# ModelCloud/GPTQModel

Hardware: NVIDIA H100
Metric: W4A16 g128 QuantLinear: decode tok/s + prefill TFLOPS vs HBM/TC roofline (higher is better)
Workload: dtype f16

## Files before the change

### gptqmodel_b200/csrc/b2q_api.cu

```cuda
#include <cstdarg>
#include <cstdio>
#include <cstdlib>

#include "../../include/b2q.h"
#include "b2q_internal.h"

namespace b2q {
static thread_local char g_err[512] = "";

void set_error(const char* fmt, ...) {
  va_list ap;
  va_start(ap, fmt);
  vsnprintf(g_err, sizeof(g_err), fmt, ap);
  va_end(ap);
}

static int env_int(const char* name, int dflt) {
  const char* e = getenv(name);
  return (e != nullptr && e[0] != 0) ? atoi(e) : dflt;
}

static EnvCfg read_env() {
  EnvCfg c;
  c.disable_pdl = env_int("B2Q_DISABLE_PDL", 0);
  c.midm = env_int("B2Q_MIDM", 1);
  c.decode_blocks_m = env_int("B2Q_DECODE_BLOCKS_M", 0);
  c.decode_groups2 = env_int("B2Q_DECODE_GROUPS", 1) == 2;
  c.decode_v2 = env_int("B2Q_DECODE_V2", -1);
  c.decode2_gw = env_int("B2Q_DECODE2_GW", 0);
  c.decode2_ks = env_int("B2Q_DECODE2_KS", 0);
  c.decode2_xtma = env_int("B2Q_DECODE2_XTMA", 0);
  c.decode2_fastsync = env_int("B2Q_DECODE2_FASTSYNC", 0);
  c.midm_ks = env_int("B2Q_MIDM_KS", 0);
  c.midm_dqg1 = env_int("B2Q_MIDM_DQG1", 0);
  return c;
}

int num_sms() {
  static int cache[32] = {};
  int dev = 0;
  if (cudaGetDevice(&dev) != cudaSuccess || dev < 0 || dev >= 32) {
    (void)cudaGetLastError();
    return 132;
  }
  if (cache[dev] == 0) {
    int n = 0;
    if (cudaDeviceGetAttribute(&n, cudaDevAttrMultiProcessorCount, dev) != cudaSuccess || n <= 0) {
      (void)cudaGetLastError();
      n = 132;
    }
    cache[dev] = n < 160 ? n : 160;
  }
  return cache[dev];
}

static EnvCfg g_env = read_env();
const EnvCfg& env() { return g_env; }
void reload_env() { g_env = read_env(); }

struct DeviceGuard {
  int prev = -1, dev = -1;
  explicit DeviceGuard(const void* p) {
    cudaPointerAttributes at;
    if (p != nullptr && cudaPointerGetAttributes(&at, p) == cudaSuccess && at.type == cudaMemoryTypeDevice) {
      dev = at.device;
      if (cudaGetDevice(&prev) == cudaSuccess && prev != dev) cudaSetDevice(dev);
      else prev = -1;
    }
    (void)cudaGetLastError();
  }
  ~DeviceGuard() {
    if (prev >= 0) cudaSetDevice(prev);
  }
};

static int check_cuda(int e, const char* what) {
  if (e > 0) set_error("%s: CUDA error %d (%s)", what, e, cudaGetErrorString((cudaError_t)e));
  return e;
}

static int validate(const char* fn, const void* x, const void* packed, const void* scales, const void* out, int M,
                    int K, int N, int bits, int group_size, int dtype) {
  if (x == nullptr || packed == nullptr || scales == nullptr || out == nullptr) {
    set_error("%s: null pointer argument", fn);
    return -2;
  }
  if (bits != 4 && bits != 8) {
// ... 467 lines not shown
```

### gptqmodel_b200/csrc/b2q_gemm.cu

```cuda
#include <cuda.h>

#include "b2q_common.cuh"
#include "b2q_dequant.cuh"
#include "b2q_gemm.cuh"
#include "b2q_internal.h"
#include "b2q_wgmma.cuh"

namespace b2q {

template <typename T, int BITS, bool ASYM, int STAGES>
__global__ void __launch_bounds__(G_THREADS, 1)
    gemm_kernel(const __grid_constant__ CUtensorMap tmap_x, const __grid_constant__ GemmSets S, int M, int K,
                int gshc) {
  using C = GemmCfg<BITS, STAGES>;
  using E = ET<T>;
  extern __shared__ uint8_t smem_raw[];
  const uint32_t smem_base = (smem_u32(smem_raw) + 1023u) & ~1023u;
  uint8_t* smem = smem_raw + (smem_base - smem_u32(smem_raw));

  const uint32_t sA = smem_base;
  const uint32_t sB = sA + STAGES * C::A_BYTES;
  const uint32_t sP = sB + STAGES * C::B_BYTES;
  const uint32_t sBar = sP + STAGES * C::P_BYTES;
  const uint32_t bar_full = sBar, bar_bready = sBar + 8 * STAGES, bar_empty = sBar + 16 * STAGES;

  int set = 0, tn = blockIdx.x;
  if (S.nsets > 1 && tn >= S.tn_end[0]) {
    set = (S.nsets > 2 && tn >= S.tn_end[1]) ? 2 : 1;
    tn -= S.tn_end[set - 1];
  }
  const int N = S.N[set];
  const uint4* __restrict__ packed = S.packed[set];
  const T* __restrict__ scales = reinterpret_cast<const T*>(S.scales[set]);
  const uint32_t* __restrict__ qzeros = S.qzeros[set];

  const int warp = threadIdx.x >> 5, lane = threadIdx.x & 31;
  const int NT = N >> 5;
  const int n0 = tn * G_BN, m0 = blockIdx.y * G_BM;
  const int nt0 = n0 >> 5;
  const int ntiles = min(4, NT - nt0);
  const int nkb = K / G_BK;

  if (threadIdx.x == 0) {
    prefetch_tmap(&tmap_x);
    for (int s = 0; s < STAGES; ++s) {
      mbar_init(bar_full + 8 * s, 1);
      mbar_init(bar_bready + 8 * s, G_DQ_THREADS);
      mbar_init(bar_empty + 8 * s, 1);
    }
    fence_mbar_init();
  }
  __syncthreads();

  if (warp == 8) {
    if (lane == 0) {
      const int FT = N >> 4, ft0 = n0 >> 4;
      const uint32_t pbytes4 = (uint32_t)min(8, FT - ft0) * 512u;
      const uint32_t pbytes8 = (uint32_t)ntiles * C::SUB * 512u;
      for (int kb = 0; kb < nkb; ++kb) {
        const int s = kb % STAGES;
        const uint32_t ph = (kb / STAGES) & 1;
        mbar_wait(bar_empty + 8 * s, ph ^ 1);
        const int g0 = (2 * kb) >> gshc, g1 = (2 * kb + 1) >> gshc;
        const int nrows = (g1 != g0) ? 2 : 1;
        const uint32_t sbytes = (uint32_t)min(G_BN, N - n0) * 2u, zbytes = ASYM ? sbytes / 4u : 0u;
        mbar_expect_tx(bar_full + 8 * s,
                       C::A_BYTES + (BITS == 4 ? pbytes4 + nrows * (sbytes + zbytes) : 2 * pbytes8));
        tma_load_2d(sA + s * C::A_BYTES, &tmap_x, bar_full + 8 * s, kb * G_BK, m0);
        if (BITS == 4) {
          bulk_load(sP + s * C::P_BYTES, packed + ((size_t)kb * FT + ft0) * 32, pbytes4, bar_full + 8 * s);
          for (int r = 0; r < nrows; ++r) {
            const int gr = r ? g1 : g0;
            bulk_load(sP + s * C::P_BYTES + 4096 + r * 320, scales + (size_t)gr * N + n0, sbytes, bar_full + 8 * s);
            if (ASYM)
              bulk_load(sP + s * C::P_BYTES + 4096 + r * 320 + 256, qzeros + (size_t)gr * (N >> 3) + (n0 >> 3),
                        zbytes, bar_full + 8 * s);
          }
        } else {
#pragma unroll
          for (int j = 0; j < 2; ++j)
            bulk_load(sP + s * C::P_BYTES + j * C::P_CHUNK_BYTES,
                      packed + ((size_t)(kb * 2 + j) * NT + nt0) * C::SUB * 32, pbytes8, bar_full + 8 * s);
        }
      }
    }
  } else if (warp < 4) {
    float acc[2][G_BN / 2];
#pragma unroll
    for (int mb = 0; mb < 2; ++mb)
#pragma unroll
      for (int i = 0; i < G_BN / 2; ++i) acc[mb][i] = 0.f;
    for (int kb = 0; kb < nkb; ++kb) {
      const int s = kb % STAGES;
      const uint32_t ph = (kb / STAGES) & 1;
      mbar_wait(bar_full + 8 * s, ph);
      mbar_wait(bar_bready + 8 * s, ph);
      wgmma_fence();
      const uint64_t bdesc = wgmma_desc_k_sw128(sB + s * C::B_BYTES);
      const uint64_t adesc = wgmma_desc_k_sw128(sA + s * C::A_BYTES);
#pragma unroll
      for (int k = 0; k < G_BK / 16; ++k) {
#pragma unroll
        for (int mb = 0; mb < 2; ++mb)
          Wgmma<E::FMT, G_BN>::mma(acc[mb], adesc + 512 * mb + 2 * k, bdesc + 2 * k, (kb | k) != 0 ? 1u : 0u);
      }
      wgmma_commit();
      wgmma_wait<1>();
      if (kb > 0 && threadIdx.x == 0) mbar_arrive(bar_empty + 8 * ((kb - 1) % STAGES));
    }
    wgmma_wait<0>();
#pragma unroll
    for (int mb = 0; mb < 2; ++mb) wgmma_fence_regs(acc[mb]);

    const T* __restrict__ bias = reinterpret_cast<const T*>(S.bias[set]);
    T* __restrict__ out = reinterpret_cast<T*>(S.out[set]);
#pragma unroll
    for (int mb = 0; mb < 2; ++mb) {
#pragma unroll
      for (int h = 0; h < 2; ++h) {
        const int row = m0 + 64 * mb + 16 * warp + (lane >> 2) + 8 * h;
        if (row >= M) continue;
        T* dst = out + (size_t)row * N;
#pragma unroll
        for (int j = 0; j < G_BN / 8; ++j) {
          const int col = n0 + 8 * j + 2 * (lane & 3);
          if (col >= N) continue;
          float f0 = acc[mb][4 * j + 2 * h], f1 = acc[mb][4 * j + 2 * h + 1];
          if (bias != nullptr) {
            f0 = E::to_f(E::from_f(f0)) + E::to_f(bias[col]);
            f1 = E::to_f(E::from_f(f1)) + E::to_f(bias[col + 1]);
          }
          *reinterpret_cast<uint32_t*>(dst + col) = E::pack2(f0, f1);
        }
      }
    }
  } else {
    const int t = threadIdx.x - G_MMA_THREADS;
    constexpr int PF = 32 / BITS;
    constexpr int ZSYM = 1 << (BITS - 1);
    if (BITS == 4) {
      const int lp = t & 31, g = lp >> 2, tt = lp & 3;
      int f[4];
      f[0] = (t >> 5) * 16 + g;
      f[1] = f[0] + 8;
      f[2] = f[0] + 64;
      f[3] = f[0] + 72;
      for (int kb = 0; kb < nkb; ++kb) {
        const int s = kb % STAGES;
        const uint32_t ph = (kb / STAGES) & 1;
        mbar_wait(bar_full + 8 * s, ph);
        const uint8_t* pst = smem + (sP - smem_base) + s * C::P_BYTES;
        const uint4* pj = reinterpret_cast<const uint4*>(pst);
        const int grow = ((2 * kb + (tt >> 1)) >> gshc) - ((2 * kb) >> gshc);
        const uint8_t* srow = pst + 4096 + grow * 320;
#pragma unroll
        for (int u = 0; u < 2; ++u) {
          const uint4 pv = pj[t + u * 128];
          const uint32_t s_lo = *reinterpret_cast<const uint16_t*>(srow + f[2 * u] * 2);
          const uint32_t s_hi = *reinterpret_cast<const uint16_t*>(srow + f[2 * u + 1] * 2);
          int zl = ZSYM, zh = ZSYM;
          if (ASYM) {
            const uint32_t zwl = *reinterpret_cast<const uint32_t*>(srow + 256 + (f[2 * u] >> 3) * 4);
            const uint32_t zwh = *reinterpret_cast<const uint32_t*>(srow + 256 + (f[2 * u + 1] >> 3) * 4);
            zl = (int)((zwl >> (4 * g)) & 15u);
            zh = (int)((zwh >> (4 * g)) & 15u);
          }
          uint4 lo[2], hi[2];
          Dequant<T, 4>::run(pv, s_lo, zl, s_hi, zh, lo, hi);
          const uint32_t sw = (uint32_t)g;
          const uint32_t rlo = sB + s * C::B_BYTES + f[2 * u] * 128;
          const uint32_t rhi = rlo + 8 * 128;
#pragma unroll
          for (int c = 0; c < 2; ++c) {
            const uint32_t off = (((uint32_t)(2 * tt + c)) ^ sw) << 4;
            asm volatile("st.shared.v4.u32 [%0], {%1,%2,%3,%4};" ::"r"(rlo + off), "r"(lo[c].x), "r"(lo[c].y),
                         "r"(lo[c].z), "r"(lo[c].w)
                         : "memory");
            asm volatile("st.shared.v4.u32 [%0], {%1,%2,%3,%4};" ::"r"(rhi + off), "r"(hi[c].x), "r"(hi[c].y),
                         "r"(hi[c].z), "r"(hi[c].w)
                         : "memory");
          }
        }
        fence_proxy_async_smem();
        mbar_arrive(bar_bready + 8 * s);
      }
    } else {
      const int n = n0 + t;
      const int nsafe = (n < N) ? n : 0;
      const int ntl = t >> 5;
      SZRaw cur[2], nxt[2];
      cur[0] = load_sz<T, BITS, ASYM>(scales, qzeros, 0, nsafe, N);
      cur[1] = load_sz<T, BITS, ASYM>(scales, qzeros, 1 >> gshc, nsafe, N);
      for (int kb = 0; kb < nkb; ++kb) {
        const int s = kb % STAGES;
        const uint32_t ph = (kb / STAGES) & 1;
        if (kb + 1 < nkb) {
          nxt[0] = load_sz<T, BITS, ASYM>(scales, qzeros, (2 * kb + 2) >> gshc, nsafe, N);
          nxt[1] = load_sz<T, BITS, ASYM>(scales, qzeros, (2 * kb + 3) >> gshc, nsafe, N);
        }
        mbar_wait(bar_full + 8 * s, ph);
        const uint32_t brow = sB + s * C::B_BYTES + t * 128;
        const uint32_t sw = (uint32_t)(t & 7);
#pragma unroll
        for (int j = 0; j < 2; ++j) {
          int z = ZSYM;
          if (ASYM) z = (int)((cur[j].zw >> (BITS * (nsafe % PF))) & ((1u << BITS) - 1));
          const uint4* pj = reinterpret_cast<const uint4*>(smem + (sP - smem_base) + s * C::P_BYTES +
                                                           j * C::P_CHUNK_BYTES);
#pragma unroll
          for (int h = 0; h < 2; ++h) {
            const uint4 pv = pj[(ntl * 2 + h) * 32 + lane];
            uint4 o[2];
            Dequant<T, 8>::run(pv, cur[j].s, z, o);
#pragma unroll
            for (int c = 0; c < 2; ++c) {
              const uint32_t addr = brow + (((uint32_t)(j * 4 + h * 2 + c) ^ sw) << 4);
              asm volatile("st.shared.v4.u32 [%0], {%1,%2,%3,%4};" ::"r"(addr), "r"(o[c].x), "r"(o[c].y),
                           "r"(o[c].z), "r"(o[c].w)
                           : "memory");
            }
          }
        }
        fence_proxy_async_smem();
        mbar_arrive(bar_bready + 8 * s);
        cur[0] = nxt[0];
        cur[1] = nxt[1];
      }
    }
  }
}

typedef CUresult (*EncodeTiledFn)(CUtensorMap*, CUtensorMapDataType, cuuint32_t, void*, const cuuint64_t*,
                                  const cuuint64_t*, const cuuint32_t*, const cuuint32_t*, CUtensorMapInterleave,
                                  CUtensorMapSwizzle, CUtensorMapL2promotion, CUtensorMapFloatOOBfill);

static EncodeTiledFn get_encode_fn() {
  static EncodeTiledFn fn = nullptr;
  if (fn == nullptr) {
    void* p = nullptr;
    cudaDriverEntryPointQueryResult qres;
    if (cudaGetDriverEntryPoint("cuTensorMapEncodeTiled", &p, cudaEnableDefault, &qres) == cudaSuccess &&
        qres == cudaDriverEntryPointSuccess)
      fn = reinterpret_cast<EncodeTiledFn>(p);
  }
  return fn;
}

int make_x_tmap_box(CUtensorMap* map, const void* x, int M, int K, int dtype, int box_rows) {
  struct Entry {
    const void* x;
    int M, K, dtype, box;
    CUtensorMap map;
  };
  constexpr int NCACHE = 16;
  static thread_local Entry cache[NCACHE];
  static thread_local int next = 0, filled = 0;
  for (int i = 0; i < filled; ++i) {
    const Entry& c = cache[i];
    if (c.x == x && c.M == M && c.K == K && c.dtype == dtype && c.box == box_rows) {
      *map = c.map;
      return 0;
    }
  }
  EncodeTiledFn enc = get_encode_fn();
  if (enc == nullptr) {
    set_error("b2q_gemm: cuTensorMapEncodeTiled not available from the driver");
    return -1;
  }
  cuuint64_t gdim[2] = {(cuuint64_t)K, (cuuint64_t)M};
  cuuint64_t gstride[1] = {(cuuint64_t)K * 2};
  cuuint32_t box[2] = {(cuuint32_t)G_BK, (cuuint32_t)box_rows};
  cuuint32_t estr[2] = {1, 1};
  CUresult r = enc(map, dtype == 0 ? CU_TENSOR_MAP_DATA_TYPE_FLOAT16 : CU_TENSOR_MAP_DATA_TYPE_BFLOAT16, 2,
                   const_cast<void*>(x), gdim, gstride, box, estr, CU_TENSOR_MAP_INTERLEAVE_NONE,
                   CU_TENSOR_MAP_SWIZZLE_128B, CU_TENSOR_MAP_L2_PROMOTION_L2_256B,
                   CU_TENSOR_MAP_FLOAT_OOB_FILL_NONE);
  if (r != CUDA_SUCCESS) {
    set_error("b2q_gemm: cuTensorMapEncodeTiled failed (%d) for x=%p M=%d K=%d box=%d", (int)r, x, M, K, box_rows);
    return -1;
  }
  Entry& e = cache[next];
  e.x = x;
  e.M = M;
  e.K = K;
  e.dtype = dtype;
  e.box = box_rows;
  e.map = *map;
  next = (next + 1) % NCACHE;
  if (filled < NCACHE) ++filled;
  return 0;
}

int make_x_tmap(CUtensorMap* map, const void* x, int M, int K, int dtype) {
  return make_x_tmap_box(map, x, M, K, dtype, 128);
}

int gemm_gshc(const MmArgs& a) {
  if (a.group_size == 32) return 0;
  if (a.group_size == 64) return 1;
  if (a.group_size == 128) return 2;
  return 31;
}


template <typename T, int BITS, bool ASYM, int STAGES>
static int launch_gemm_t(const MmArgs& a, const void* x, const GemmSets& S) {
  using C = GemmCfg<BITS, STAGES>;
  CUtensorMap tmap;
  if (make_x_tmap(&tmap, x, a.M, a.K, a.dtype) != 0) return -1;
  auto kern = gemm_kernel<T, BITS, ASYM, STAGES>;
  static uint32_t smem_ok = 0;
  if (int e = ensure_dyn_smem(kern, C::SMEM_BYTES, smem_ok, "b2q_gemm")) return e;
  dim3 grid(S.tn_end[S.nsets - 1], (a.M + G_BM - 1) / G_BM, 1);
  kern<<<grid, G_THREADS, C::SMEM_BYTES, a.stream>>>(tmap, S, a.M, a.K, gemm_gshc(a));
  return (int)cudaGetLastError();
}

static int launch_gemm_sets(const MmArgs& a, const void* x, const GemmSets& S) {
  const bool asym = S.qzeros[0] != nullptr;
#define B2Q_GEMM_CASE(T, BITS, ST) \
  (asym ? launch_gemm_t<T, BITS, true, ST>(a, x, S) : launch_gemm_t<T, BITS, false, ST>(a, x, S))
  if (a.dtype == 0) return a.bits == 4 ? B2Q_GEMM_CASE(__half, 4, 4) : B2Q_GEMM_CASE(__half, 8, 4);
  return a.bits == 4 ? B2Q_GEMM_CASE(__nv_bfloat16, 4, 4) : B2Q_GEMM_CASE(__nv_bfloat16, 8, 4);
#undef B2Q_GEMM_CASE
}

int launch_gemm_multi(const MmArgs& a, const void* x, int nsets, const void* const* packed, const void* const* scales,
                      const int32_t* const* qzeros, const void* const* bias, void* const* out, const int* Ns) {
  if (nsets < 1 || nsets > G_MAX_SETS) {
    set_error("b2q_gemm_multi: nsets=%d out of range (1..%d)", nsets, G_MAX_SETS);
    return -1;
  }
  if (a.K % G_BK != 0) {
    set_error("b2q_gemm_multi: K=%d must be a multiple of %d", a.K, G_BK);
    return -1;
  }
  GemmSets S = {};
  S.nsets = nsets;
  int tn = 0;
  for (int i = 0; i < nsets; ++i) {
    if (Ns[i] <= 0 || Ns[i] % 32 != 0 || packed[i] == nullptr || scales[i] == nullptr || out[i] == nullptr ||
        ((qzeros[i] != nullptr) != (qzeros[0] != nullptr))) {
      set_error("b2q_gemm_multi: set %d unsupported (N=%d; all sets share K, group size and symmetry)", i, Ns[i]);
      return -1;
    }
    tn += (Ns[i] + G_BN - 1) / G_BN;
    S.tn_end[i] = tn;
    S.N[i] = Ns[i];
    S.packed[i] = (const uint4*)packed[i];
    S.scales[i] = scales[i];
    S.qzeros[i] = (const uint32_t*)qzeros[i];
    S.bias[i] = bias[i];
    S.out[i] = out[i];
  }
  for (int i = nsets; i < G_MAX_SETS; ++i) S.tn_end[i] = tn;
  return launch_gemm_sets(a, x, S);
}

int launch_gemm(const MmArgs& a) {
  if (a.K % G_BK != 0) {
    set_error("b2q_gemm: K=%d must be a multiple of %d", a.K, G_BK);
    return -1;
  }
  const void* x = a.x;
  if (a.perm != nullptr) {
    const size_t need = (size_t)a.M * a.K * 2;
    if (a.workspace == nullptr || a.workspace_bytes < need) {
      set_error("b2q_gemm: act-order needs a %zu-byte workspace (got %zu)", need, a.workspace_bytes);
      return -1;
    }
    int e = launch_permute_cols(a.x, a.perm, a.workspace, a.M, a.K, a.stream);
    if (e != 0) return e;
    x = a.workspace;
  }
  if (a.M <= 128 && env().midm && midm_supported(a)) return launch_midm(a, x);
  const void* packed = a.packed;
  const void* scales = a.scales;
  const int32_t* qzeros = (const int32_t*)a.qzeros;
  const void* bias = a.bias;
  void* out = a.out;
  return launch_gemm_multi(a, x, 1, &packed, &scales, &qzeros, &bias, &out, &a.N);
}

}
```

### gptqmodel_b200/csrc/b2q_gemm.cuh

```cuda
#pragma once
#include "b2q_common.cuh"

namespace b2q {

constexpr int G_BM = 128;
constexpr int G_BN = 128;
constexpr int G_BK = 64;
constexpr int G_MMA_THREADS = 128;
constexpr int G_DQ_THREADS = 128;
constexpr int G_THREADS = G_MMA_THREADS + G_DQ_THREADS + 32;

template <int BITS, int STAGES>
struct GemmCfg {
  static constexpr int SUB = BITS / 4;
  static constexpr int A_BYTES = G_BM * G_BK * 2;
  static constexpr int B_BYTES = G_BN * G_BK * 2;
  static constexpr int P_CHUNK_BYTES = 4 * SUB * 512;
  static constexpr int P_BYTES = 2 * P_CHUNK_BYTES + (BITS == 4 ? 1024 : 0);
  static constexpr int STAGE_BYTES = A_BYTES + B_BYTES + P_BYTES;
  static constexpr int BAR_BYTES = 256;
  static constexpr int SMEM_BYTES = STAGES * STAGE_BYTES + BAR_BYTES + 1024;
  static_assert(SMEM_BYTES <= 227 * 1024, "dynamic shared memory of one CTA");
};

constexpr int G_MAX_SETS = 3;
struct GemmSets {
  int nsets;
  int tn_end[G_MAX_SETS];
  int N[G_MAX_SETS];
  const uint4* packed[G_MAX_SETS];
  const void* scales[G_MAX_SETS];
  const uint32_t* qzeros[G_MAX_SETS];
  const void* bias[G_MAX_SETS];
  void* out[G_MAX_SETS];
};

}
```

### gptqmodel_b200/csrc/b2q_internal.h

```cpp
#pragma once
#include <cuda_runtime.h>
#include <stdint.h>

namespace b2q {

int num_sms();

struct MmArgs {
  const void* x;
  const void* packed;
  const void* scales;
  const void* qzeros;
  const int32_t* perm;
  const void* bias;
  void* out;
  int M, K, N;
  int bits;
  int group_size;
  int dtype;
  void* workspace;
  size_t workspace_bytes;
  cudaStream_t stream;
  int tune_ks;
  int tune_warps;
// ... 15 lines not shown
int launch_gemv(const MmArgs& a);
int launch_decode(const MmArgs& a);
bool decode_supported(const MmArgs& a);
bool decode_plan(int version, const MmArgs& a, int NT, int* out8);
int launch_decode_multi(const MmArgs& a, int nsets, const void* const* packed, const void* const* scales,
                        const int32_t* const* qzeros, const void* const* bias, void* const* out, const int* Ns);
int launch_gemm(const MmArgs& a);
bool midm_supported(const MmArgs& a);
int midm_ranks(int K, int N);
int launch_midm(const MmArgs& a, const void* x);
struct MoeGroupedArgs {
  const int32_t* counts;
  const int32_t* offsets;
  const int32_t* sorted_pairs;
  const float* pair_weights;
  const void* packed3;
  const void* scales3;
  const void* qzeros3;
  float* ypair;
  int E, rows, active;
};
int launch_midm_grouped(int mode, const MmArgs& a, const MoeGroupedArgs& g);
int launch_moe_align(const int32_t* topk_ids, int T, int top_k, int E, int32_t* counts, int32_t* offsets,
                     int32_t* sorted_pairs, cudaStream_t stream);
int launch_moe_gather(const void* x, const int32_t* sorted_pairs, void* xs, int rows, int top_k, int K,
                      cudaStream_t stream);
int launch_moe_gather_perm(const void* src, const int32_t* sorted_pairs, const int32_t* perms, const int32_t* offsets,
                           int E, void* dst, int rows, int top_k, int K, cudaStream_t stream);
int launch_moe_combine(const float* ypair, void* y, int T, int top_k, int N, int dtype, cudaStream_t stream);
int launch_moe_decode_gate_up(const MmArgs& a, const void* packed1, const void* scales1, const int32_t* qzeros1,
                              const void* packed3, const void* scales3, const int32_t* qzeros3, const int32_t* ids,
                              int top_k, int E, void* gu);
int launch_moe_decode_act(const void* gu, void* h, int top_k, int N, int dtype, cudaStream_t stream);
int launch_moe_decode_down(const MmArgs& a, const int32_t* ids, const float* wts, int top_k, int E, int fused_act);
int launch_gemm_multi(const MmArgs& a, const void* x, int nsets, const void* const* packed, const void* const* scales,
                      const int32_t* const* qzeros, const void* const* bias, void* const* out, const int* Ns);
int gemm_gshc(const MmArgs& a);
int launch_allreduce(void* inout, int n, int dtype, int rank, int world, const void* const* peer_bufs,
                     size_t flag_offset, int max_elems, void* seq, cudaStream_t stream);
void set_error(const char* fmt, ...);

struct EnvCfg {
  int disable_pdl;
  int midm;
  int decode_blocks_m;
  int decode_groups2;
  int decode_v2;
  int decode2_gw;
  int decode2_ks;
  int decode2_xtma;
  int decode2_fastsync;
  int midm_ks;
  int midm_dqg1;
};
const EnvCfg& env();
void reload_env();

template <typename Kern>
inline int ensure_dyn_smem(Kern kern, int bytes, uint32_t& done_mask, const char* who) {
  int dev = 0;
  cudaGetDevice(&dev);
  if (dev < 32 && ((done_mask >> dev) & 1u)) return 0;
  cudaError_t e = cudaFuncSetAttribute(kern, cudaFuncAttributeMaxDynamicSharedMemorySize, bytes);
  if (e != cudaSuccess) {
    set_error("%s: cannot opt in to %d bytes of shared memory: %s", who, bytes, cudaGetErrorString(e));
    return (int)e;
  }
  if (dev < 32) done_mask |= 1u << dev;
  return 0;
}
extern void* g_trace_ptr;

}
```

### gptqmodel_b200/csrc/b2q_wgmma.cuh

```cuda
#pragma once
#include "b2q_common.cuh"

namespace b2q {

__device__ __forceinline__ uint64_t wgmma_desc_k_sw128(uint32_t saddr) {
  return (uint64_t)((saddr & 0x3FFFFu) >> 4) | (1ull << 16) | (64ull << 32) | (1ull << 62);
}
__device__ __forceinline__ void wgmma_fence() { asm volatile("wgmma.fence.sync.aligned;" ::: "memory"); }
__device__ __forceinline__ void wgmma_commit() { asm volatile("wgmma.commit_group.sync.aligned;" ::: "memory"); }
template <int N>
__device__ __forceinline__ void wgmma_wait() {
  asm volatile("wgmma.wait_group.sync.aligned %0;" ::"n"(N) : "memory");
}
template <int R>
__device__ __forceinline__ void wgmma_fence_regs(float (&d)[R]) {
#pragma unroll
  for (int i = 0; i < R; ++i) asm volatile("" : "+f"(d[i])::"memory");
}

template <int FMT, int N>
struct Wgmma;
template <>
struct Wgmma<0, 16> {
  __device__ static __forceinline__ void mma(float (&d)[8], uint64_t a, uint64_t b, uint32_t accumulate) {
// ... 25 lines not shown
  }
};
template <>
struct Wgmma<0, 128> {
  __device__ static __forceinline__ void mma(float (&d)[64], uint64_t a, uint64_t b, uint32_t accumulate) {
    asm volatile(
        "{ .reg .pred p; setp.ne.b32 p, %66, 0;\n"
        "  wgmma.mma_async.sync.aligned.m64n128k16.f32.f16.f16 {%0,%1,%2,%3,%4,%5,%6,%7,%8,%9,%10,%11,%12,%13,%14,%15,%16,%17,%18,%19,%20,%21,%22,%23,%24,%25,%26,%27,%28,%29,%30,%31,%32,%33,%34,%35,%36,%37,%38,%39,%40,%41,%42,%43,%44,%45,%46,%47,%48,%49,%50,%51,%52,%53,%54,%55,%56,%57,%58,%59,%60,%61,%62,%63}, %64, %65, p, 1, 1, 0, 0; }"
        : "+f"(d[0]), "+f"(d[1]), "+f"(d[2]), "+f"(d[3]), "+f"(d[4]), "+f"(d[5]), "+f"(d[6]), "+f"(d[7]), "+f"(d[8]), "+f"(d[9]), "+f"(d[10]), "+f"(d[11]), "+f"(d[12]), "+f"(d[13]), "+f"(d[14]), "+f"(d[15]), "+f"(d[16]), "+f"(d[17]), "+f"(d[18]), "+f"(d[19]), "+f"(d[20]), "+f"(d[21]), "+f"(d[22]), "+f"(d[23]), "+f"(d[24]), "+f"(d[25]), "+f"(d[26]), "+f"(d[27]), "+f"(d[28]), "+f"(d[29]), "+f"(d[30]), "+f"(d[31]), "+f"(d[32]), "+f"(d[33]), "+f"(d[34]), "+f"(d[35]), "+f"(d[36]), "+f"(d[37]), "+f"(d[38]), "+f"(d[39]), "+f"(d[40]), "+f"(d[41]), "+f"(d[42]), "+f"(d[43]), "+f"(d[44]), "+f"(d[45]), "+f"(d[46]), "+f"(d[47]), "+f"(d[48]), "+f"(d[49]), "+f"(d[50]), "+f"(d[51]), "+f"(d[52]), "+f"(d[53]), "+f"(d[54]), "+f"(d[55]), "+f"(d[56]), "+f"(d[57]), "+f"(d[58]), "+f"(d[59]), "+f"(d[60]), "+f"(d[61]), "+f"(d[62]), "+f"(d[63])
        : "l"(a), "l"(b), "r"(accumulate));
  }
};
template <>
struct Wgmma<1, 16> {
  __device__ static __forceinline__ void mma(float (&d)[8], uint64_t a, uint64_t b, uint32_t accumulate) {
    asm volatile(
        "{ .reg .pred p; setp.ne.b32 p, %10, 0;\n"
        "  wgmma.mma_async.sync.aligned.m64n16k16.f32.bf16.bf16 {%0,%1,%2,%3,%4,%5,%6,%7}, %8, %9, p, 1, 1, 0, 0; }"
        : "+f"(d[0]), "+f"(d[1]), "+f"(d[2]), "+f"(d[3]), "+f"(d[4]), "+f"(d[5]), "+f"(d[6]), "+f"(d[7])
        : "l"(a), "l"(b), "r"(accumulate));
  }
};
template <>
struct Wgmma<1, 32> {
  __device__ static __forceinline__ void mma(float (&d)[16], uint64_t a, uint64_t b, uint32_t accumulate) {
    asm volatile(
        "{ .reg .pred p; setp.ne.b32 p, %18, 0;\n"
        "  wgmma.mma_async.sync.aligned.m64n32k16.f32.bf16.bf16 {%0,%1,%2,%3,%4,%5,%6,%7,%8,%9,%10,%11,%12,%13,%14,%15}, %16, %17, p, 1, 1, 0, 0; }"
        : "+f"(d[0]), "+f"(d[1]), "+f"(d[2]), "+f"(d[3]), "+f"(d[4]), "+f"(d[5]), "+f"(d[6]), "+f"(d[7]), "+f"(d[8]), "+f"(d[9]), "+f"(d[10]), "+f"(d[11]), "+f"(d[12]), "+f"(d[13]), "+f"(d[14]), "+f"(d[15])
        : "l"(a), "l"(b), "r"(accumulate));
  }
};
template <>
struct Wgmma<1, 64> {
  __device__ static __forceinline__ void mma(float (&d)[32], uint64_t a, uint64_t b, uint32_t accumulate) {
    asm volatile(
        "{ .reg .pred p; setp.ne.b32 p, %34, 0;\n"
        "  wgmma.mma_async.sync.aligned.m64n64k16.f32.bf16.bf16 {%0,%1,%2,%3,%4,%5,%6,%7,%8,%9,%10,%11,%12,%13,%14,%15,%16,%17,%18,%19,%20,%21,%22,%23,%24,%25,%26,%27,%28,%29,%30,%31}, %32, %33, p, 1, 1, 0, 0; }"
        : "+f"(d[0]), "+f"(d[1]), "+f"(d[2]), "+f"(d[3]), "+f"(d[4]), "+f"(d[5]), "+f"(d[6]), "+f"(d[7]), "+f"(d[8]), "+f"(d[9]), "+f"(d[10]), "+f"(d[11]), "+f"(d[12]), "+f"(d[13]), "+f"(d[14]), "+f"(d[15]), "+f"(d[16]), "+f"(d[17]), "+f"(d[18]), "+f"(d[19]), "+f"(d[20]), "+f"(d[21]), "+f"(d[22]), "+f"(d[23]), "+f"(d[24]), "+f"(d[25]), "+f"(d[26]), "+f"(d[27]), "+f"(d[28]), "+f"(d[29]), "+f"(d[30]), "+f"(d[31])
        : "l"(a), "l"(b), "r"(accumulate));
  }
};
template <>
struct Wgmma<1, 128> {
  __device__ static __forceinline__ void mma(float (&d)[64], uint64_t a, uint64_t b, uint32_t accumulate) {
    asm volatile(
        "{ .reg .pred p; setp.ne.b32 p, %66, 0;\n"
        "  wgmma.mma_async.sync.aligned.m64n128k16.f32.bf16.bf16 {%0,%1,%2,%3,%4,%5,%6,%7,%8,%9,%10,%11,%12,%13,%14,%15,%16,%17,%18,%19,%20,%21,%22,%23,%24,%25,%26,%27,%28,%29,%30,%31,%32,%33,%34,%35,%36,%37,%38,%39,%40,%41,%42,%43,%44,%45,%46,%47,%48,%49,%50,%51,%52,%53,%54,%55,%56,%57,%58,%59,%60,%61,%62,%63}, %64, %65, p, 1, 1, 0, 0; }"
        : "+f"(d[0]), "+f"(d[1]), "+f"(d[2]), "+f"(d[3]), "+f"(d[4]), "+f"(d[5]), "+f"(d[6]), "+f"(d[7]), "+f"(d[8]), "+f"(d[9]), "+f"(d[10]), "+f"(d[11]), "+f"(d[12]), "+f"(d[13]), "+f"(d[14]), "+f"(d[15]), "+f"(d[16]), "+f"(d[17]), "+f"(d[18]), "+f"(d[19]), "+f"(d[20]), "+f"(d[21]), "+f"(d[22]), "+f"(d[23]), "+f"(d[24]), "+f"(d[25]), "+f"(d[26]), "+f"(d[27]), "+f"(d[28]), "+f"(d[29]), "+f"(d[30]), "+f"(d[31]), "+f"(d[32]), "+f"(d[33]), "+f"(d[34]), "+f"(d[35]), "+f"(d[36]), "+f"(d[37]), "+f"(d[38]), "+f"(d[39]), "+f"(d[40]), "+f"(d[41]), "+f"(d[42]), "+f"(d[43]), "+f"(d[44]), "+f"(d[45]), "+f"(d[46]), "+f"(d[47]), "+f"(d[48]), "+f"(d[49]), "+f"(d[50]), "+f"(d[51]), "+f"(d[52]), "+f"(d[53]), "+f"(d[54]), "+f"(d[55]), "+f"(d[56]), "+f"(d[57]), "+f"(d[58]), "+f"(d[59]), "+f"(d[60]), "+f"(d[61]), "+f"(d[62]), "+f"(d[63])
        : "l"(a), "l"(b), "r"(accumulate));
  }
};

}
```

Before: 583.9.

## Use two consumer warpgroups with BN up to 256 and banded tile rasterization

The prefill GEMM changes from one MMA warpgroup that issues two m64 wgmmas per k-step to two MMA warpgroups, each owning 64 rows, with a new N=256 tile option and 3 stages. A heuristic based on wave quantization picks between BN 128 and 256. Tiles now go on a 1D grid in bands of 16 M-tiles so concurrent CTAs share the same weight and activation tiles in L2. Dequant warps drop to 3, striding over the fragment tiles, which may make B dequantization the bottleneck at BN=256 and raises register pressure (128 fp32 accumulators per thread).

```diff
diff --git a/gptqmodel_b200/csrc/b2q_api.cu b/gptqmodel_b200/csrc/b2q_api.cu
--- a/gptqmodel_b200/csrc/b2q_api.cu
+++ b/gptqmodel_b200/csrc/b2q_api.cu
@@ -33,6 +33,7 @@
   c.decode2_fastsync = env_int("B2Q_DECODE2_FASTSYNC", 0);
   c.midm_ks = env_int("B2Q_MIDM_KS", 0);
   c.midm_dqg1 = env_int("B2Q_MIDM_DQG1", 0);
+  c.gemm_bn = env_int("B2Q_GEMM_BN", 0);
   return c;
 }
 
diff --git a/gptqmodel_b200/csrc/b2q_gemm.cu b/gptqmodel_b200/csrc/b2q_gemm.cu
--- a/gptqmodel_b200/csrc/b2q_gemm.cu
+++ b/gptqmodel_b200/csrc/b2q_gemm.cu
@@ -8,11 +8,12 @@
 
 namespace b2q {
 
-template <typename T, int BITS, bool ASYM, int STAGES>
+template <typename T, int BITS, bool ASYM, int BN>
 __global__ void __launch_bounds__(G_THREADS, 1)
     gemm_kernel(const __grid_constant__ CUtensorMap tmap_x, const __grid_constant__ GemmSets S, int M, int K,
                 int gshc) {
-  using C = GemmCfg<BITS, STAGES>;
+  using C = GemmCfg<BITS, BN>;
+  constexpr int STAGES = C::STAGES;
   using E = ET<T>;
   extern __shared__ uint8_t smem_raw[];
   const uint32_t smem_base = (smem_u32(smem_raw) + 1023u) & ~1023u;
@@ -24,7 +25,12 @@
   const uint32_t sBar = sP + STAGES * C::P_BYTES;
   const uint32_t bar_full = sBar, bar_bready = sBar + 8 * STAGES, bar_empty = sBar + 16 * STAGES;
 
-  int set = 0, tn = blockIdx.x;
+  const int MT = (M + G_BM - 1) / G_BM, TN = S.tn_end[S.nsets - 1];
+  const int band = blockIdx.x / (G_BAND * TN);
+  const int mt0 = band * G_BAND, bm = min(G_BAND, MT - mt0);
+  const int rem = blockIdx.x - band * G_BAND * TN;
+  const int m0 = (mt0 + rem % bm) * G_BM;
+  int set = 0, tn = rem / bm;
   if (S.nsets > 1 && tn >= S.tn_end[0]) {
     set = (S.nsets > 2 && tn >= S.tn_end[1]) ? 2 : 1;
     tn -= S.tn_end[set - 1];
@@ -36,9 +42,8 @@
 
   const int warp = threadIdx.x >> 5, lane = threadIdx.x & 31;
   const int NT = N >> 5;
-  const int n0 = tn * G_BN, m0 = blockIdx.y * G_BM;
+  const int n0 = tn * BN;
   const int nt0 = n0 >> 5;
-  const int ntiles = min(4, NT - nt0);
   const int nkb = K / G_BK;
 
   if (threadIdx.x == 0) {
@@ -46,24 +51,24 @@
     for (int s = 0; s < STAGES; ++s) {
       mbar_init(bar_full + 8 * s, 1);
       mbar_init(bar_bready + 8 * s, G_DQ_THREADS);
-      mbar_init(bar_empty + 8 * s, 1);
+      mbar_init(bar_empty + 8 * s, 2);
     }
     fence_mbar_init();
   }
   __syncthreads();
 
-  if (warp == 8) {
+  if (warp == 11) {
     if (lane == 0) {
       const int FT = N >> 4, ft0 = n0 >> 4;
-      const uint32_t pbytes4 = (uint32_t)min(8, FT - ft0) * 512u;
-      const uint32_t pbytes8 = (uint32_t)ntiles * C::SUB * 512u;
+      const uint32_t pbytes4 = (uint32_t)min(BN / 16, FT - ft0) * 512u;
+      const uint32_t pbytes8 = (uint32_t)min(BN / 32, NT - nt0) * 1024u;
       for (int kb = 0; kb < nkb; ++kb) {
         const int s = kb % STAGES;
         const uint32_t ph = (kb / STAGES) & 1;
         mbar_wait(bar_empty + 8 * s, ph ^ 1);
         const int g0 = (2 * kb) >> gshc, g1 = (2 * kb + 1) >> gshc;
         const int nrows = (g1 != g0) ? 2 : 1;
-        const uint32_t sbytes = (uint32_t)min(G_BN, N - n0) * 2u, zbytes = ASYM ? sbytes / 4u : 0u;
+        const uint32_t sbytes = (uint32_t)min(BN, N - n0) * 2u, zbytes = ASYM ? sbytes / 4u : 0u;
         mbar_expect_tx(bar_full + 8 * s,
                        C::A_BYTES + (BITS == 4 ? pbytes4 + nrows * (sbytes + zbytes) : 2 * pbytes8));
         tma_load_2d(sA + s * C::A_BYTES, &tmap_x, bar_full + 8 * s, kb * G_BK, m0);
@@ -71,25 +76,24 @@
           bulk_load(sP + s * C::P_BYTES, packed + ((size_t)kb * FT + ft0) * 32, pbytes4, bar_full + 8 * s);
           for (int r = 0; r < nrows; ++r) {
             const int gr = r ? g1 : g0;
-            bulk_load(sP + s * C::P_BYTES + 4096 + r * 320, scales + (size_t)gr * N + n0, sbytes, bar_full + 8 * s);
+            const uint32_t srow = sP + s * C::P_BYTES + C::PK_BYTES + r * C::SROW_BYTES;
+            bulk_load(srow, scales + (size_t)gr * N + n0, sbytes, bar_full + 8 * s);
             if (ASYM)
-              bulk_load(sP + s * C::P_BYTES + 4096 + r * 320 + 256, qzeros + (size_t)gr * (N >> 3) + (n0 >> 3),
-                        zbytes, bar_full + 8 * s);
+              bulk_load(srow + BN * 2, qzeros + (size_t)gr * (N >> 3) + (n0 >> 3), zbytes, bar_full + 8 * s);
           }
         } else {
 #pragma unroll
           for (int j = 0; j < 2; ++j)
             bulk_load(sP + s * C::P_BYTES + j * C::P_CHUNK_BYTES,
-                      packed + ((size_t)(kb * 2 + j) * NT + nt0) * C::SUB * 32, pbytes8, bar_full + 8 * s);
+                      packed + ((size_t)(kb * 2 + j) * NT + nt0) * 64, pbytes8, bar_full + 8 * s);
         }
       }
     }
-  } else if (warp < 4) {
-    float acc[2][G_BN / 2];
-#pragma unroll
-    for (int mb = 0; mb < 2; ++mb)
-#pragma unroll
-      for (int i = 0; i < G_BN / 2; ++i) acc[mb][i] = 0.f;
+  } else if (warp < 8) {
+    const int wg = warp >> 2;
+    float acc[BN / 2];
+#pragma unroll
+    for (int i = 0; i < BN / 2; ++i) acc[i] = 0.f;
     for (int kb = 0; kb < nkb; ++kb) {
       const int s = kb % STAGES;
       const uint32_t ph = (kb / STAGES) & 1;
@@ -97,54 +101,42 @@
       mbar_wait(bar_bready + 8 * s, ph);
       wgmma_fence();
       const uint64_t bdesc = wgmma_desc_k_sw128(sB + s * C::B_BYTES);
-      const uint64_t adesc = wgmma_desc_k_sw128(sA + s * C::A_BYTES);
-#pragma unroll
-      for (int k = 0; k < G_BK / 16; ++k) {
-#pragma unroll
-        for (int mb = 0; mb < 2; ++mb)
-          Wgmma<E::FMT, G_BN>::mma(acc[mb], adesc + 512 * mb + 2 * k, bdesc + 2 * k, (kb | k) != 0 ? 1u : 0u);
-      }
+      const uint64_t adesc = wgmma_desc_k_sw128(sA + s * C::A_BYTES) + 512 * wg;
+#pragma unroll
+      for (int k = 0; k < G_BK / 16; ++k)
+        Wgmma<E::FMT, BN>::mma(acc, adesc + 2 * k, bdesc + 2 * k, (kb | k) != 0 ? 1u : 0u);
       wgmma_commit();
       wgmma_wait<1>();
-      if (kb > 0 && threadIdx.x == 0) mbar_arrive(bar_empty + 8 * ((kb - 1) % STAGES));
+      if (kb > 0 && (threadIdx.x & 127) == 0) mbar_arrive(bar_empty + 8 * ((kb - 1) % STAGES));
     }
     wgmma_wait<0>();
-#pragma unroll
-    for (int mb = 0; mb < 2; ++mb) wgmma_fence_regs(acc[mb]);
+    wgmma_fence_regs(acc);
 
     const T* __restrict__ bias = reinterpret_cast<const T*>(S.bias[set]);
     T* __restrict__ out = reinterpret_cast<T*>(S.out[set]);
 #pragma unroll
-    for (int mb = 0; mb < 2; ++mb) {
-#pragma unroll
-      for (int h = 0; h < 2; ++h) {
-        const int row = m0 + 64 * mb + 16 * warp + (lane >> 2) + 8 * h;
-        if (row >= M) continue;
-        T* dst = out + (size_t)row * N;
-#pragma unroll
-        for (int j = 0; j < G_BN / 8; ++j) {
-          const int col = n0 + 8 * j + 2 * (lane & 3);
-          if (col >= N) continue;
-          float f0 = acc[mb][4 * j + 2 * h], f1 = acc[mb][4 * j + 2 * h + 1];
-          if (bias != nullptr) {
-            f0 = E::to_f(E::from_f(f0)) + E::to_f(bias[col]);
-            f1 = E::to_f(E::from_f(f1)) + E::to_f(bias[col + 1]);
-          }
-          *reinterpret_cast<uint32_t*>(dst + col) = E::pack2(f0, f1);
-        }
+    for (int h = 0; h < 2; ++h) {
+      const int row = m0 + 16 * warp + (lane >> 2) + 8 * h;
+      if (row >= M) continue;
+      T* dst = out + (size_t)row * N;
+#pragma unroll
+      for (int j = 0; j < BN / 8; ++j) {
+        const int col = n0 + 8 * j + 2 * (lane & 3);
+        if (col >= N) continue;
+        float f0 = acc[4 * j + 2 * h], f1 = acc[4 * j + 2 * h + 1];
+        if (bias != nullptr) {
+          f0 = E::to_f(E::from_f(f0)) + E::to_f(bias[col]);
+          f1 = E::to_f(E::from_f(f1)) + E::to_f(bias[col + 1]);
+        }
+        *reinterpret_cast<uint32_t*>(dst + col) = E::pack2(f0, f1);
       }
     }
   } else {
-    const int t = threadIdx.x - G_MMA_THREADS;
+    const int dw = warp - 8;
     constexpr int PF = 32 / BITS;
     constexpr int ZSYM = 1 << (BITS - 1);
     if (BITS == 4) {
-      const int lp = t & 31, g = lp >> 2, tt = lp & 3;
-      int f[4];
-      f[0] = (t >> 5) * 16 + g;
-      f[1] = f[0] + 8;
-      f[2] = f[0] + 64;
-      f[3] = f[0] + 72;
+      const int g = lane >> 2, tt = lane & 3;
       for (int kb = 0; kb < nkb; ++kb) {
         const int s = kb % STAGES;
         const uint32_t ph = (kb / STAGES) & 1;
@@ -152,23 +144,24 @@
         const uint8_t* pst = smem + (sP - smem_base) + s * C::P_BYTES;
         const uint4* pj = reinterpret_cast<const uint4*>(pst);
         const int grow = ((2 * kb + (tt >> 1)) >> gshc) - ((2 * kb) >> gshc);
-        const uint8_t* srow = pst + 4096 + grow * 320;
-#pragma unroll
-        for (int u = 0; u < 2; ++u) {
-          const uint4 pv = pj[t + u * 128];
-          const uint32_t s_lo = *reinterpret_cast<const uint16_t*>(srow + f[2 * u] * 2);
-          const uint32_t s_hi = *reinterpret_cast<const uint16_t*>(srow + f[2 * u + 1] * 2);
+        const uint8_t* srow = pst + C::PK_BYTES + grow * C::SROW_BYTES;
+#pragma unroll
+        for (int ft = dw; ft < BN / 16; ft += 3) {
+          const int flo = 16 * ft + g, fhi = flo + 8;
+          const uint4 pv = pj[32 * ft + lane];
+          const uint32_t s_lo = *reinterpret_cast<const uint16_t*>(srow + flo * 2);
+          const uint32_t s_hi = *reinterpret_cast<const uint16_t*>(srow + fhi * 2);
           int zl = ZSYM, zh = ZSYM;
           if (ASYM) {
-            const uint32_t zwl = *reinterpret_cast<const uint32_t*>(srow + 256 + (f[2 * u] >> 3) * 4);
-            const uint32_t zwh = *reinterpret_cast<const uint32_t*>(srow + 256 + (f[2 * u + 1] >> 3) * 4);
+            const uint32_t zwl = *reinterpret_cast<const uint32_t*>(srow + BN * 2 + (flo >> 3) * 4);
+            const uint32_t zwh = *reinterpret_cast<const uint32_t*>(srow + BN * 2 + (fhi >> 3) * 4);
             zl = (int)((zwl >> (4 * g)) & 15u);
             zh = (int)((zwh >> (4 * g)) & 15u);
           }
           uint4 lo[2], hi[2];
           Dequant<T, 4>::run(pv, s_lo, zl, s_hi, zh, lo, hi);
           const uint32_t sw = (uint32_t)g;
-          const uint32_t rlo = sB + s * C::B_BYTES + f[2 * u] * 128;
+          const uint32_t rlo = sB + s * C::B_BYTES + flo * 128;
           const uint32_t rhi = rlo + 8 * 128;
 #pragma unroll
           for (int c = 0; c < 2; ++c) {
@@ -185,46 +178,61 @@
         mbar_arrive(bar_bready + 8 * s);
       }
     } else {
-      const int n = n0 + t;
-      const int nsafe = (n < N) ? n : 0;
-      const int ntl = t >> 5;
-      SZRaw cur[2], nxt[2];
-      cur[0] = load_sz<T, BITS, ASYM>(scales, qzeros, 0, nsafe, N);
-      cur[1] = load_sz<T, BITS, ASYM>(scales, qzeros, 1 >> gshc, nsafe, N);
+      constexpr int NV = (BN / 32 + 2) / 3;
+      int nsafe[NV];
+      SZRaw cur[NV][2], nxt[NV][2];
+#pragma unroll
+      for (int v = 0; v < NV; ++v) {
+        const int n = n0 + 32 * (dw + 3 * v) + lane;
+        nsafe[v] = (n < N) ? n : 0;
+        cur[v][0] = load_sz<T, BITS, ASYM>(scales, qzeros, 0, nsafe[v], N);
+        cur[v][1] = load_sz<T, BITS, ASYM>(scales, qzeros, 1 >> gshc, nsafe[v], N);
+      }
       for (int kb = 0; kb < nkb; ++kb) {
         const int s = kb % STAGES;
         const uint32_t ph = (kb / STAGES) & 1;
         if (kb + 1 < nkb) {
-          nxt[0] = load_sz<T, BITS, ASYM>(scales, qzeros, (2 * kb + 2) >> gshc, nsafe, N);
-          nxt[1] = load_sz<T, BITS, ASYM>(scales, qzeros, (2 * kb + 3) >> gshc, nsafe, N);
+#pragma unroll
+          for (int v = 0; v < NV; ++v) {
+            nxt[v][0] = load_sz<T, BITS, ASYM>(scales, qzeros, (2 * kb + 2) >> gshc, nsafe[v], N);
+            nxt[v][1] = load_sz<T, BITS, ASYM>(scales, qzeros, (2 * kb + 3) >> gshc, nsafe[v], N);
+          }
         }
         mbar_wait(bar_full + 8 * s, ph);
-        const uint32_t brow = sB + s * C::B_BYTES + t * 128;
-        const uint32_t sw = (uint32_t)(t & 7);
-#pragma unroll
-        for (int j = 0; j < 2; ++j) {
-          int z = ZSYM;
-          if (ASYM) z = (int)((cur[j].zw >> (BITS * (nsafe % PF))) & ((1u << BITS) - 1));
-          const uint4* pj = reinterpret_cast<const uint4*>(smem + (sP - smem_base) + s * C::P_BYTES +
-                                                           j * C::P_CHUNK_BYTES);
-#pragma unroll
-          for (int h = 0; h < 2; ++h) {
-            const uint4 pv = pj[(ntl * 2 + h) * 32 + lane];
-            uint4 o[2];
-            Dequant<T, 8>::run(pv, cur[j].s, z, o);
-#pragma unroll
-            for (int c = 0; c < 2; ++c) {
-              const uint32_t addr = brow + (((uint32_t)(j * 4 + h * 2 + c) ^ sw) << 4);
-              asm volatile("st.shared.v4.u32 [%0], {%1,%2,%3,%4};" ::"r"(addr), "r"(o[c].x), "r"(o[c].y),
-                           "r"(o[c].z), "r"(o[c].w)
-                           : "memory");
+        const uint32_t sw = (uint32_t)(lane & 7);
+#pragma unroll
+        for (int v = 0; v < NV; ++v) {
+          const int ntl = dw + 3 * v;
+          if (ntl >= BN / 32) break;
+          const uint32_t brow = sB + s * C::B_BYTES + (32 * ntl + lane) * 128;
+#pragma unroll
+          for (int j = 0; j < 2; ++j) {
+            int z = ZSYM;
+            if (ASYM) z = (int)((cur[v][j].zw >> (BITS * (nsafe[v] % PF))) & ((1u << BITS) - 1));
+            const uint4* pj = reinterpret_cast<const uint4*>(smem + (sP - smem_base) + s * C::P_BYTES +
+                                                             j * C::P_CHUNK_BYTES);
+#pragma unroll
+            for (int h = 0; h < 2; ++h) {
+              const uint4 pv = pj[(ntl * 2 + h) * 32 + lane];
+              uint4 o[2];
+              Dequant<T, 8>::run(pv, cur[v][j].s, z, o);
+#pragma unroll
+              for (int c = 0; c < 2; ++c) {
+                const uint32_t addr = brow + (((uint32_t)(j * 4 + h * 2 + c) ^ sw) << 4);
+                asm volatile("st.shared.v4.u32 [%0], {%1,%2,%3,%4};" ::"r"(addr), "r"(o[c].x), "r"(o[c].y),
+                             "r"(o[c].z), "r"(o[c].w)
+                             : "memory");
+              }
             }
           }
         }
         fence_proxy_async_smem();
         mbar_arrive(bar_bready + 8 * s);
-        cur[0] = nxt[0];
-        cur[1] = nxt[1];
+#pragma unroll
+        for (int v = 0; v < NV; ++v) {
+          cur[v][0] = nxt[v][0];
+          cur[v][1] = nxt[v][1];
+        }
       }
     }
   }
@@ -303,26 +311,45 @@
 }
 
 
-template <typename T, int BITS, bool ASYM, int STAGES>
+template <typename T, int BITS, bool ASYM, int BN>
 static int launch_gemm_t(const MmArgs& a, const void* x, const GemmSets& S) {
-  using C = GemmCfg<BITS, STAGES>;
+  using C = GemmCfg<BITS, BN>;
   CUtensorMap tmap;
   if (make_x_tmap(&tmap, x, a.M, a.K, a.dtype) != 0) return -1;
-  auto kern = gemm_kernel<T, BITS, ASYM, STAGES>;
+  auto kern = gemm_kernel<T, BITS, ASYM, BN>;
   static uint32_t smem_ok = 0;
   if (int e = ensure_dyn_smem(kern, C::SMEM_BYTES, smem_ok, "b2q_gemm")) return e;
-  dim3 grid(S.tn_end[S.nsets - 1], (a.M + G_BM - 1) / G_BM, 1);
-  kern<<<grid, G_THREADS, C::SMEM_BYTES, a.stream>>>(tmap, S, a.M, a.K, gemm_gshc(a));
+  const long long ctas = (long long)S.tn_end[S.nsets - 1] * ((a.M + G_BM - 1) / G_BM);
+  if (ctas > 0x7fffffffLL) {
+    set_error("b2q_gemm: %lld tiles exceed the grid limit (M=%d)", ctas, a.M);
+    return -1;
+  }
+  kern<<<(unsigned)ctas, G_THREADS, C::SMEM_BYTES, a.stream>>>(tmap, S, a.M, a.K, gemm_gshc(a));
   return (int)cudaGetLastError();
 }
 
-static int launch_gemm_sets(const MmArgs& a, const void* x, const GemmSets& S) {
+template <int BN>
+static int launch_gemm_bn(const MmArgs& a, const void* x, const GemmSets& S) {
   const bool asym = S.qzeros[0] != nullptr;
-#define B2Q_GEMM_CASE(T, BITS, ST) \
-  (asym ? launch_gemm_t<T, BITS, true, ST>(a, x, S) : launch_gemm_t<T, BITS, false, ST>(a, x, S))
-  if (a.dtype == 0) return a.bits == 4 ? B2Q_GEMM_CASE(__half, 4, 4) : B2Q_GEMM_CASE(__half, 8, 4);
-  return a.bits == 4 ? B2Q_GEMM_CASE(__nv_bfloat16, 4, 4) : B2Q_GEMM_CASE(__nv_bfloat16, 8, 4);
+#define B2Q_GEMM_CASE(T, BITS) \
+  (asym ? launch_gemm_t<T, BITS, true, BN>(a, x, S) : launch_gemm_t<T, BITS, false, BN>(a, x, S))
+  if (a.dtype == 0) return a.bits == 4 ? B2Q_GEMM_CASE(__half, 4) : B2Q_GEMM_CASE(__half, 8);
+  return a.bits == 4 ? B2Q_GEMM_CASE(__nv_bfloat16, 4) : B2Q_GEMM_CASE(__nv_bfloat16, 8);
 #undef B2Q_GEMM_CASE
+}
+
+constexpr double G_BN128_COST = 1.15;
+
+int gemm_bn(int M, int nsets, const int* Ns) {
+  if (env().gemm_bn == 128 || env().gemm_bn == 256) return env().gemm_bn;
+  const long long mt = (M + G_BM - 1) / G_BM, sms = num_sms();
+  long long t128 = 0, t256 = 0;
+  for (int i = 0; i < nsets; ++i) {
+    t128 += (Ns[i] + 127) / 128;
+    t256 += (Ns[i] + 255) / 256;
+  }
+  const long long w128 = (t128 * mt + sms - 1) / sms, w256 = (t256 * mt + sms - 1) / sms;
+  return (double)w256 * 256.0 <= (double)w128 * 128.0 * G_BN128_COST ? 256 : 128;
 }
 
 int launch_gemm_multi(const MmArgs& a, const void* x, int nsets, const void* const* packed, const void* const* scales,
@@ -335,16 +362,19 @@
     set_error("b2q_gemm_multi: K=%d must be a multiple of %d", a.K, G_BK);
     return -1;
   }
-  GemmSets S = {};
-  S.nsets = nsets;
-  int tn = 0;
   for (int i = 0; i < nsets; ++i) {
     if (Ns[i] <= 0 || Ns[i] % 32 != 0 || packed[i] == nullptr || scales[i] == nullptr || out[i] == nullptr ||
         ((qzeros[i] != nullptr) != (qzeros[0] != nullptr))) {
       set_error("b2q_gemm_multi: set %d unsupported (N=%d; all sets share K, group size and symmetry)", i, Ns[i]);
       return -1;
     }
-    tn += (Ns[i] + G_BN - 1) / G_BN;
+  }
+  const int bn = gemm_bn(a.M, nsets, Ns);
+  GemmSets S = {};
+  S.nsets = nsets;
+  int tn = 0;
+  for (int i = 0; i < nsets; ++i) {
+    tn += (Ns[i] + bn - 1) / bn;
     S.tn_end[i] = tn;
     S.N[i] = Ns[i];
     S.packed[i] = (const uint4*)packed[i];
@@ -354,7 +384,7 @@
     S.out[i] = out[i];
   }
   for (int i = nsets; i < G_MAX_SETS; ++i) S.tn_end[i] = tn;
-  return launch_gemm_sets(a, x, S);
+  return bn == 256 ? launch_gemm_bn<256>(a, x, S) : launch_gemm_bn<128>(a, x, S);
 }
 
 int launch_gemm(const MmArgs& a) {
diff --git a/gptqmodel_b200/csrc/b2q_gemm.cuh b/gptqmodel_b200/csrc/b2q_gemm.cuh
--- a/gptqmodel_b200/csrc/b2q_gemm.cuh
+++ b/gptqmodel_b200/csrc/b2q_gemm.cuh
@@ -4,19 +4,21 @@
 namespace b2q {
 
 constexpr int G_BM = 128;
-constexpr int G_BN = 128;
 constexpr int G_BK = 64;
-constexpr int G_MMA_THREADS = 128;
-constexpr int G_DQ_THREADS = 128;
+constexpr int G_MMA_THREADS = 256;
+constexpr int G_DQ_THREADS = 96;
 constexpr int G_THREADS = G_MMA_THREADS + G_DQ_THREADS + 32;
+constexpr int G_BAND = 16;
 
-template <int BITS, int STAGES>
+template <int BITS, int BN>
 struct GemmCfg {
-  static constexpr int SUB = BITS / 4;
+  static constexpr int STAGES = BN == 256 ? 3 : 4;
   static constexpr int A_BYTES = G_BM * G_BK * 2;
-  static constexpr int B_BYTES = G_BN * G_BK * 2;
-  static constexpr int P_CHUNK_BYTES = 4 * SUB * 512;
-  static constexpr int P_BYTES = 2 * P_CHUNK_BYTES + (BITS == 4 ? 1024 : 0);
+  static constexpr int B_BYTES = BN * G_BK * 2;
+  static constexpr int PK_BYTES = BN * G_BK * BITS / 8;
+  static constexpr int P_CHUNK_BYTES = PK_BYTES / 2;
+  static constexpr int SROW_BYTES = BN * 2 + BN / 2;
+  static constexpr int P_BYTES = PK_BYTES + (BITS == 4 ? 2 * SROW_BYTES : 0);
   static constexpr int STAGE_BYTES = A_BYTES + B_BYTES + P_BYTES;
   static constexpr int BAR_BYTES = 256;
   static constexpr int SMEM_BYTES = STAGES * STAGE_BYTES + BAR_BYTES + 1024;
diff --git a/gptqmodel_b200/csrc/b2q_internal.h b/gptqmodel_b200/csrc/b2q_internal.h
--- a/gptqmodel_b200/csrc/b2q_internal.h
+++ b/gptqmodel_b200/csrc/b2q_internal.h
@@ -91,6 +91,7 @@
   int decode2_fastsync;
   int midm_ks;
   int midm_dqg1;
+  int gemm_bn;
 };
 const EnvCfg& env();
 void reload_env();
diff --git a/gptqmodel_b200/csrc/b2q_wgmma.cuh b/gptqmodel_b200/csrc/b2q_wgmma.cuh
--- a/gptqmodel_b200/csrc/b2q_wgmma.cuh
+++ b/gptqmodel_b200/csrc/b2q_wgmma.cuh
@@ -101,4 +101,25 @@
   }
 };
 
+template <>
+struct Wgmma<0, 256> {
+  __device__ static __forceinline__ void mma(float (&d)[128], uint64_t a, uint64_t b, uint32_t accumulate) {
+    asm volatile(
+        "{ .reg .pred p; setp.ne.b32 p, %130, 0;\n"
+        "  wgmma.mma_async.sync.aligned.m64n256k16.f32.f16.f16 {%0,%1,%2,%3,%4,%5,%6,%7,%8,%9,%10,%11,%12,%13,%14,%15,%16,%17,%18,%19,%20,%21,%22,%23,%24,%25,%26,%27,%28,%29,%30,%31,%32,%33,%34,%35,%36,%37,%38,%39,%40,%41,%42,%43,%44,%45,%46,%47,%48,%49,%50,%51,%52,%53,%54,%55,%56,%57,%58,%59,%60,%61,%62,%63,%64,%65,%66,%67,%68,%69,%70,%71,%72,%73,%74,%75,%76,%77,%78,%79,%80,%81,%82,%83,%84,%85,%86,%87,%88,%89,%90,%91,%92,%93,%94,%95,%96,%97,%98,%99,%100,%101,%102,%103,%104,%105,%106,%107,%108,%109,%110,%111,%112,%113,%114,%115,%116,%117,%118,%119,%120,%121,%122,%123,%124,%125,%126,%127}, %128, %129, p, 1, 1, 0, 0; }"
+        : "+f"(d[0]), "+f"(d[1]), "+f"(d[2]), "+f"(d[3]), "+f"(d[4]), "+f"(d[5]), "+f"(d[6]), "+f"(d[7]), "+f"(d[8]), "+f"(d[9]), "+f"(d[10]), "+f"(d[11]), "+f"(d[12]), "+f"(d[13]), "+f"(d[14]), "+f"(d[15]), "+f"(d[16]), "+f"(d[17]), "+f"(d[18]), "+f"(d[19]), "+f"(d[20]), "+f"(d[21]), "+f"(d[22]), "+f"(d[23]), "+f"(d[24]), "+f"(d[25]), "+f"(d[26]), "+f"(d[27]), "+f"(d[28]), "+f"(d[29]), "+f"(d[30]), "+f"(d[31]), "+f"(d[32]), "+f"(d[33]), "+f"(d[34]), "+f"(d[35]), "+f"(d[36]), "+f"(d[37]), "+f"(d[38]), "+f"(d[39]), "+f"(d[40]), "+f"(d[41]), "+f"(d[42]), "+f"(d[43]), "+f"(d[44]), "+f"(d[45]), "+f"(d[46]), "+f"(d[47]), "+f"(d[48]), "+f"(d[49]), "+f"(d[50]), "+f"(d[51]), "+f"(d[52]), "+f"(d[53]), "+f"(d[54]), "+f"(d[55]), "+f"(d[56]), "+f"(d[57]), "+f"(d[58]), "+f"(d[59]), "+f"(d[60]), "+f"(d[61]), "+f"(d[62]), "+f"(d[63]), "+f"(d[64]), "+f"(d[65]), "+f"(d[66]), "+f"(d[67]), "+f"(d[68]), "+f"(d[69]), "+f"(d[70]), "+f"(d[71]), "+f"(d[72]), "+f"(d[73]), "+f"(d[74]), "+f"(d[75]), "+f"(d[76]), "+f"(d[77]), "+f"(d[78]), "+f"(d[79]), "+f"(d[80]), "+f"(d[81]), "+f"(d[82]), "+f"(d[83]), "+f"(d[84]), "+f"(d[85]), "+f"(d[86]), "+f"(d[87]), "+f"(d[88]), "+f"(d[89]), "+f"(d[90]), "+f"(d[91]), "+f"(d[92]), "+f"(d[93]), "+f"(d[94]), "+f"(d[95]), "+f"(d[96]), "+f"(d[97]), "+f"(d[98]), "+f"(d[99]), "+f"(d[100]), "+f"(d[101]), "+f"(d[102]), "+f"(d[103]), "+f"(d[104]), "+f"(d[105]), "+f"(d[106]), "+f"(d[107]), "+f"(d[108]), "+f"(d[109]), "+f"(d[110]), "+f"(d[111]), "+f"(d[112]), "+f"(d[113]), "+f"(d[114]), "+f"(d[115]), "+f"(d[116]), "+f"(d[117]), "+f"(d[118]), "+f"(d[119]), "+f"(d[120]), "+f"(d[121]), "+f"(d[122]), "+f"(d[123]), "+f"(d[124]), "+f"(d[125]), "+f"(d[126]), "+f"(d[127])
+        : "l"(a), "l"(b), "r"(accumulate));
+  }
+};
+template <>
+struct Wgmma<1, 256> {
+  __device__ static __forceinline__ void mma(float (&d)[128], uint64_t a, uint64_t b, uint32_t accumulate) {
+    asm volatile(
+        "{ .reg .pred p; setp.ne.b32 p, %130, 0;\n"
+        "  wgmma.mma_async.sync.aligned.m64n256k16.f32.bf16.bf16 {%0,%1,%2,%3,%4,%5,%6,%7,%8,%9,%10,%11,%12,%13,%14,%15,%16,%17,%18,%19,%20,%21,%22,%23,%24,%25,%26,%27,%28,%29,%30,%31,%32,%33,%34,%35,%36,%37,%38,%39,%40,%41,%42,%43,%44,%45,%46,%47,%48,%49,%50,%51,%52,%53,%54,%55,%56,%57,%58,%59,%60,%61,%62,%63,%64,%65,%66,%67,%68,%69,%70,%71,%72,%73,%74,%75,%76,%77,%78,%79,%80,%81,%82,%83,%84,%85,%86,%87,%88,%89,%90,%91,%92,%93,%94,%95,%96,%97,%98,%99,%100,%101,%102,%103,%104,%105,%106,%107,%108,%109,%110,%111,%112,%113,%114,%115,%116,%117,%118,%119,%120,%121,%122,%123,%124,%125,%126,%127}, %128, %129, p, 1, 1, 0, 0; }"
+        : "+f"(d[0]), "+f"(d[1]), "+f"(d[2]), "+f"(d[3]), "+f"(d[4]), "+f"(d[5]), "+f"(d[6]), "+f"(d[7]), "+f"(d[8]), "+f"(d[9]), "+f"(d[10]), "+f"(d[11]), "+f"(d[12]), "+f"(d[13]), "+f"(d[14]), "+f"(d[15]), "+f"(d[16]), "+f"(d[17]), "+f"(d[18]), "+f"(d[19]), "+f"(d[20]), "+f"(d[21]), "+f"(d[22]), "+f"(d[23]), "+f"(d[24]), "+f"(d[25]), "+f"(d[26]), "+f"(d[27]), "+f"(d[28]), "+f"(d[29]), "+f"(d[30]), "+f"(d[31]), "+f"(d[32]), "+f"(d[33]), "+f"(d[34]), "+f"(d[35]), "+f"(d[36]), "+f"(d[37]), "+f"(d[38]), "+f"(d[39]), "+f"(d[40]), "+f"(d[41]), "+f"(d[42]), "+f"(d[43]), "+f"(d[44]), "+f"(d[45]), "+f"(d[46]), "+f"(d[47]), "+f"(d[48]), "+f"(d[49]), "+f"(d[50]), "+f"(d[51]), "+f"(d[52]), "+f"(d[53]), "+f"(d[54]), "+f"(d[55]), "+f"(d[56]), "+f"(d[57]), "+f"(d[58]), "+f"(d[59]), "+f"(d[60]), "+f"(d[61]), "+f"(d[62]), "+f"(d[63]), "+f"(d[64]), "+f"(d[65]), "+f"(d[66]), "+f"(d[67]), "+f"(d[68]), "+f"(d[69]), "+f"(d[70]), "+f"(d[71]), "+f"(d[72]), "+f"(d[73]), "+f"(d[74]), "+f"(d[75]), "+f"(d[76]), "+f"(d[77]), "+f"(d[78]), "+f"(d[79]), "+f"(d[80]), "+f"(d[81]), "+f"(d[82]), "+f"(d[83]), "+f"(d[84]), "+f"(d[85]), "+f"(d[86]), "+f"(d[87]), "+f"(d[88]), "+f"(d[89]), "+f"(d[90]), "+f"(d[91]), "+f"(d[92]), "+f"(d[93]), "+f"(d[94]), "+f"(d[95]), "+f"(d[96]), "+f"(d[97]), "+f"(d[98]), "+f"(d[99]), "+f"(d[100]), "+f"(d[101]), "+f"(d[102]), "+f"(d[103]), "+f"(d[104]), "+f"(d[105]), "+f"(d[106]), "+f"(d[107]), "+f"(d[108]), "+f"(d[109]), "+f"(d[110]), "+f"(d[111]), "+f"(d[112]), "+f"(d[113]), "+f"(d[114]), "+f"(d[115]), "+f"(d[116]), "+f"(d[117]), "+f"(d[118]), "+f"(d[119]), "+f"(d[120]), "+f"(d[121]), "+f"(d[122]), "+f"(d[123]), "+f"(d[124]), "+f"(d[125]), "+f"(d[126]), "+f"(d[127])
+        : "l"(a), "l"(b), "r"(accumulate));
+  }
+};
+
 }
```

Result: no change. 585.4, median of 6 (+0.3%).
